# qasimyu/simuscop

Measured on AMD Instinct MI355X. Metric: simulated paired reads/sec (whole node) at 30x WGS PE150, higher is better.
Workload: dtype u32

## Files before the change

include/simuscop_amd.h:

```cpp
#ifndef SIMUSCOP_AMD_H
#define SIMUSCOP_AMD_H

#include <stdint.h>

#ifdef __cplusplus
extern "C" {
#endif

#define SG_OK 0
#define SG_ERR_INVALID 1
#define SG_ERR_HIP 2
#define SG_ERR_UNSUPPORTED 3
#define SG_ERR_OVERFLOW 4
#define SG_ERR_FORMAT 5

#define SG_MAX_EVENTS 32

typedef struct sg_ctx sg_ctx;

int sg_create(sg_ctx** ctx, int device, uint64_t seed);
void sg_destroy(sg_ctx* ctx);
void sg_release_cached_memory(void);
const char* sg_last_error(const sg_ctx* ctx);
int sg_set_stream(sg_ctx* ctx, void* hip_stream);
// ... 301 lines not shown
int sg_train_feed_bgzf(sg_ctx* ctx, const void* members, uint64_t bytes);
int sg_train_bam_info(sg_ctx* ctx, uint64_t* records, uint64_t* inflated_bytes, double* seconds);

int sg_emit_variant(sg_ctx* ctx);
#define SG_EMIT_STRAIGHT_LINE 1
#define SG_EMIT_GENERIC_K3_LDS 2
#define SG_EMIT_GENERIC_LDS 3
#define SG_EMIT_GENERIC_GLOBAL 4
typedef struct sg_emit_path_info {
  int32_t main_kernel;
  int32_t slow_rows_lds;
  uint32_t lds_bytes;
  uint32_t clean_cap;
} sg_emit_path_info;
int sg_emit_path(const sg_ctx* ctx, sg_emit_path_info* info);

uint64_t sg_cdf_count_le(double c);

int sg_sub_row_identity_first(const double cdf4[4], int cd, uint64_t cum[3], uint8_t order[4]);
uint32_t sg_row_symbols(const double* cdf, int n);
int sg_alias_row(const double* cdf, int n, uint32_t lgW, uint32_t* thr, uint8_t* lo, uint8_t* hi);

#define SG_VCF_SKIP 0
#define SG_VCF_SNV 1
#define SG_VCF_INS 2
#define SG_VCF_DEL 3
#define SG_VCF_MALFORMED 4
#define SG_VCF_UNDECIDED 5
#define SG_VCF_HOMO 1u
#define SG_VCF_KNOWN 2u
// ... 36 lines not shown
```

simuscop_amd/__init__.py:

```python
from __future__ import annotations

import ctypes as C
import os

PKG_DIR = os.path.dirname(os.path.abspath(__file__))
LIB_DIR = os.path.join(PKG_DIR, "lib")
ENGINE_SO = os.path.join(LIB_DIR, "libsimuscop_amd.so")
HOST_SO = os.path.join(LIB_DIR, "libsimuscop_host.so")
SIMUREADS = os.path.join(LIB_DIR, "simuReads")

SG_K_NAMES = ["plan", "namebase", "indel", "scan", "emit", "emit_slow"]

ENGINE_SYMBOLS = [
    "sg_create", "sg_destroy", "sg_last_error", "sg_set_stream", "sg_set_seed", "sg_set_strict_bases", "sg_load_profile",
    "sg_upload_haplotypes", "sg_reference_begin", "sg_reference_chunk", "sg_sync", "sg_reference_scan",
    "sg_reference_commit", "sg_build_haplotypes", "sg_haplotype_codes", "sg_compress", "sg_fetch_compressed", "sg_deflate_bgzf",
    "sg_bgzf_eof", "sg_deflate_plan", "sg_detach_outputs", "sg_outputs_sizes", "sg_outputs_fetch",
    "sg_outputs_last_error", "sg_release_outputs", "sg_plan", "sg_sample", "sg_result", "sg_fetch", "sg_device_output",
    "sg_gc_percent", "sg_set_profiling", "sg_kernel_times", "sg_emit_info", "sg_emit_variant", "sg_emit_path", "sg_cdf_count_le", "sg_fetch_range", "sg_host_alloc",
    "sg_sub_row_identity_first", "sg_row_symbols", "sg_alias_row", "sg_window_weights", "sg_windows_build", "sg_plan_windows", "sg_plan_range", "sg_windows_drop",
    "sg_host_free", "sg_profile_prepare", "sg_profile_tables_error", "sg_load_prepared_profile", "sg_profile_tables_free", "sg_train_count",
    "sg_train_begin", "sg_train_feed", "sg_train_capped", "sg_train_finish", "sg_train_end",
    "sg_bgzf_members", "sg_inflate_bgzf", "sg_train_bam_start", "sg_train_feed_bgzf", "sg_train_bam_info",
    "sg_release_cached_memory",
    "sg_truth_align", "sg_truth_map", "sg_truth_pieces", "sg_truth_reads", "sg_truth_bam", "sg_fetch_truth", "sg_truth_info",
    "sg_truth_bam_tags", "sg_truth_tag_info", "sg_truth_tags",
    "sg_bamsort_pass", "sg_bamsort_merge", "sg_bamsort_index", "sg_bamsort_fetch",
    "sg_bamindex_begin", "sg_bamindex_add", "sg_bamindex_chunks", "sg_bamindex_finish", "sg_bamindex_end",
    "sg_depth_begin", "sg_depth_add", "sg_depth_add_spans", "sg_depth_bins", "sg_depth_runs", "sg_depth_fetch", "sg_depth_reset",
    "sg_depth_info", "sg_depth_end",
    "sg_variants_begin", "sg_variants_add", "sg_variants_counts", "sg_variants_reset", "sg_variants_info", "sg_variants_end",
    "sg_variant_observe",
    "sg_errtab_begin", "sg_errtab_add", "sg_errtab_counts", "sg_errtab_reset", "sg_errtab_info", "sg_errtab_end", "sg_errtab_observe",
    "sg_vcf_begin", "sg_vcf_feed", "sg_vcf_feed_bgzf", "sg_vcf_undecided", "sg_vcf_finish", "sg_vcf_rows", "sg_vcf_end", "sg_vcf_row",
# ... 22 lines not shown

class SgProfileCdf(C.Structure):
    _fields_ = [("n_bases", C.c_int32), ("bases", C.c_char * 8), ("kmer", C.c_int32), ("bins", C.c_int32),
                ("read_length", C.c_int32), ("n_qual", C.c_int32), ("min_qual", C.c_int32),
                ("insert_rate", C.c_double), ("del_rate", C.c_double),
                ("ins_cdf", C.POINTER(C.c_double)), ("n_ins", C.c_int32),
                ("del_cdf", C.POINTER(C.c_double)), ("n_del", C.c_int32),
                ("subs_cdf1", C.POINTER(C.c_double)), ("subs_cdf2", C.POINTER(C.c_double)),
                ("qual_cdf", C.POINTER(C.c_double)), ("isize_cdf", C.POINTER(C.c_double)),
                ("n_isize", C.c_int32), ("isize_min", C.c_int32), ("insert_size", C.c_int32)]


class SgWindow(C.Structure):
    _fields_ = [("hap_base", C.c_uint64), ("chain", C.c_uint32), ("spos", C.c_uint32), ("len", C.c_uint32),
                ("n_reads", C.c_int32), ("seg", C.c_uint32), ("slot_base", C.c_uint32)]


class SgBatch(C.Structure):
    _fields_ = [("batch_id", C.c_uint32), ("paired", C.c_int32), ("name_prefix", C.c_char_p),
                ("windows", C.POINTER(SgWindow)), ("n_windows", C.c_uint64),
                ("seg_size", C.POINTER(C.c_uint32)), ("seg_first_window", C.POINTER(C.c_uint32)),
                ("n_segs", C.c_uint32), ("first_window", C.c_uint32), ("first_slot", C.c_uint32)]


class SgGcWindow(C.Structure):
    _fields_ = [("start", C.c_uint64), ("chain", C.c_uint32), ("len", C.c_uint32)]


class SgGcModel(C.Structure):
    _fields_ = [("means", C.POINTER(C.c_double)), ("std", C.c_double), ("quantiles", C.POINTER(C.c_double)), ("lg_cells", C.c_uint32),
# ... 175 lines not shown
    lib.sg_gc_percent.argtypes = [vp, C.POINTER(SgGcWindow), C.c_uint64, C.POINTER(C.c_int32)]
    lib.sg_window_weights.argtypes = [vp, C.POINTER(SgGcWindow), C.POINTER(C.c_uint32), C.POINTER(C.c_uint32), C.c_uint64, C.POINTER(SgGcModel),
                                      C.POINTER(C.c_double), C.POINTER(C.c_int32)]
    lib.sg_windows_build.argtypes = [vp, C.c_uint32, C.POINTER(SgWindowGen), C.c_uint64, C.c_uint32, C.POINTER(SgGcModel), C.POINTER(C.c_double),
                                     C.POINTER(C.c_uint64)]
    lib.sg_plan_windows.argtypes = [vp, C.c_uint32, C.POINTER(SgWindowGen), C.c_uint64, C.POINTER(SgActiveSeg), C.c_uint32, C.c_uint32, C.c_uint32,
                                    C.c_int32, C.c_char_p, C.POINTER(C.c_uint64), C.POINTER(C.c_uint64)]
    lib.sg_plan_range.argtypes = [vp, C.c_uint32, C.c_uint32]
    lib.sg_windows_drop.argtypes = [vp]
    lib.sg_windows_drop.restype = None
    lib.sg_set_profiling.argtypes = [vp, C.c_int]
    lib.sg_kernel_times.argtypes = [vp, C.POINTER(C.c_float)]
    lib.sg_emit_info.argtypes = [vp, C.POINTER(C.c_uint64), C.POINTER(C.c_int)]
    lib.sg_emit_variant.argtypes = [vp]
    lib.sg_emit_path.argtypes = [vp, C.POINTER(SgEmitPathInfo)]
    lib.sg_cdf_count_le.argtypes = [C.c_double]
    lib.sg_cdf_count_le.restype = C.c_uint64
    lib.sg_sub_row_identity_first.argtypes = [C.POINTER(C.c_double), C.c_int, C.POINTER(C.c_uint64), C.POINTER(C.c_uint8)]
    lib.sg_row_symbols.argtypes = [C.POINTER(C.c_double), C.c_int]
    lib.sg_row_symbols.restype = C.c_uint32
    lib.sg_alias_row.argtypes = [C.POINTER(C.c_double), C.c_int, C.c_uint32, C.POINTER(C.c_uint32), C.POINTER(C.c_uint8),
                                 C.POINTER(C.c_uint8)]
    lib.sg_truth_align.argtypes = [C.POINTER(SgTruthPiece), C.c_uint64, C.c_uint64, C.c_uint32, C.c_int, C.POINTER(C.c_uint32), C.c_uint32,
                                   C.POINTER(C.c_int32), C.POINTER(C.c_int64), C.POINTER(C.c_uint32), C.c_uint32, C.POINTER(C.c_uint32)]
    lib.sg_truth_map.argtypes = [vp, C.POINTER(SgHapPiece), C.c_char_p, C.c_uint64, C.POINTER(C.c_int32), C.c_uint32]
    lib.sg_truth_pieces.argtypes = [vp, C.c_uint32, C.POINTER(SgTruthPiece), C.c_uint64, C.POINTER(C.c_uint64)]
    lib.sg_truth_reads.argtypes = [vp, C.c_int, C.c_uint32, C.c_uint32, C.POINTER(SgTruthRead)]
    lib.sg_truth_bam.argtypes = [vp, C.POINTER(C.c_uint64), C.POINTER(C.c_uint64)]
    lib.sg_fetch_truth.argtypes = [vp, C.c_int, C.c_uint64, C.c_uint64, C.c_char_p]
    lib.sg_truth_info.argtypes = [vp, C.POINTER(C.c_uint64), C.POINTER(C.c_uint64)]
# ... 809 lines not shown
```

simuscop_amd/csrc/sg_api.cpp:

```cpp
#include <algorithm>
#include <cstdlib>
#include <cstring>

#include "sg_api.h"
#include "sg_profile_tables.h"

thread_local std::string g_create_error;

struct sg_outputs {
  int device = 0;
  hipStream_t stream = nullptr;
  OutputSet bufs;
  uint64_t text_bytes[2] = {0, 0}, gz_bytes[2] = {0, 0};
  std::string err;
  ~sg_outputs() {
    if (stream) { (void)hipStreamSynchronize(stream); (void)hipStreamDestroy(stream); }
  }
};

sg_ctx::~sg_ctx() {
  (void)hipSetDevice(device);
  if (stream) (void)hipStreamSynchronize(stream);
  for (sg_outputs* o : spare) delete o;
  if (evs_created)
    for (auto& ev : evs) (void)hipEventDestroy(ev);
  if (own_stream) { (void)hipStreamSynchronize(own_stream); (void)hipStreamDestroy(own_stream); }
  if (mail) (void)hipHostFree(mail);
}

int finish_plan(sg_ctx* ctx, uint64_t nw, uint32_t n_segs, uint32_t n_slots, uint32_t batch_id, uint32_t first_window,
                       uint32_t first_slot, int32_t paired, const char* name_prefix) {
  const size_t plen = name_prefix ? strlen(name_prefix) : 0;
  const uint32_t nm = paired ? 2 : 1;
  SG_ENSURE(ctx->prefix, plen + 16);
  SG_ENSURE(ctx->pairs, ((size_t)n_slots + 1) * sizeof(sg::PairRec));
  SG_ENSURE(ctx->win_actual, (nw + 1) * 4);
  SG_ENSURE(ctx->win_namebase, (nw + 1) * 4);
  SG_ENSURE(ctx->events, ((size_t)nm * n_slots + 1) * 4 * SG_MAX_EVENTS);
  SG_ENSURE(ctx->recoff, ((size_t)nm * n_slots + 1) * 4);
  SG_ENSURE(ctx->meta, ((size_t)nm * n_slots + 1) * 48);
  SG_ENSURE(ctx->totals, sg::kTotalsBytes);
  SG_ENSURE(ctx->bsum, ((size_t)nm * ((n_slots + 255) / 256) + 1) * 8);
  SG_HIP(hipMemcpyAsync(ctx->prefix.p, name_prefix, plen, hipMemcpyHostToDevice, ctx->stream));
  SG_HIP(hipStreamSynchronize(ctx->stream));

  sg::DevBatch& B = ctx->B;
  B.windows = ctx->windows.as<sg_window>();
  B.n_windows = nw;
  B.seg_size = ctx->segmeta.as<uint32_t>();
  B.seg_first_window = ctx->segmeta.as<uint32_t>() + n_segs;
  B.n_segs = n_segs;
  B.n_slots = n_slots;
  B.batch_id = batch_id;
  B.win_offset = first_window;
  B.slot_offset = first_slot;
  B.paired = paired ? 1 : 0;
  B.prefix = ctx->prefix.as<uint8_t>();
  B.prefix_len = (uint32_t)plen;
  for (int i = 0; i < 4; i++) B.prefix_w[i] = 0;
  for (size_t i = 0; i < plen && i < 16; i++) B.prefix_w[i / 4] |= (uint32_t)(uint8_t)name_prefix[i] << (8 * (i % 4));
  B.pairs = ctx->pairs.as<sg::PairRec>();
  B.win_actual = ctx->win_actual.as<uint32_t>();
  B.win_namebase = ctx->win_namebase.as<uint32_t>();
  B.events = ctx->events.as<uint32_t>();
  B.recloc = ctx->recoff.as<uint32_t>();
  B.blkbase = ctx->bsum.as<uint64_t>();
  B.seg_shift = sg::record_seg_shift((uint32_t)n_slots);
// ... 275 lines not shown
    uint64_t planned = x.n_reads <= 0 ? 0 : (b->paired ? ((uint64_t)x.n_reads + 1) / 2 : (uint64_t)x.n_reads);
    slots += planned;
    if (slots > 0xFFFFFFF0ull) return ctx->fail(SG_ERR_INVALID, "sg_plan: more than 2^32 fragments in one batch");
  }
  for (uint32_t s = 0; s < b->n_segs; s++)
    if (b->seg_first_window[s] > b->seg_first_window[s + 1] || b->seg_first_window[s + 1] > nw)
      return ctx->fail(SG_ERR_INVALID, "sg_plan: seg_first_window not monotone");
  if (b->n_segs && (b->seg_first_window[0] != 0 || b->seg_first_window[b->n_segs] != nw))
    return ctx->fail(SG_ERR_INVALID, "sg_plan: seg_first_window must cover all windows");
  const size_t plen = b->name_prefix ? strlen(b->name_prefix) : 0;
  if (plen == 0 || plen > 990) return ctx->fail(SG_ERR_INVALID, "sg_plan: bad name_prefix (1..990 bytes)");
  for (uint64_t w = 0; w < nw; w++) {
    const sg_window& x = b->windows[w];
    if (x.chain >= ctx->hap.len.size()) return ctx->fail(SG_ERR_INVALID, "sg_plan: window.chain out of range");
    if (x.hap_base + x.spos + x.len > ctx->hap.len[x.chain]) return ctx->fail(SG_ERR_INVALID, "sg_plan: window runs past its chain");
  }
  SG_ENSURE(ctx->windows, (nw + 1) * sizeof(sg_window));
  SG_ENSURE(ctx->segmeta, ((size_t)b->n_segs * 2 + 2) * 4);
  if (nw) SG_HIP(hipMemcpyAsync(ctx->windows.p, b->windows, nw * sizeof(sg_window), hipMemcpyHostToDevice, ctx->stream));
  if (b->n_segs) {
    SG_HIP(hipMemcpyAsync(ctx->segmeta.p, b->seg_size, (size_t)b->n_segs * 4, hipMemcpyHostToDevice, ctx->stream));
    SG_HIP(hipMemcpyAsync(ctx->segmeta.as<uint32_t>() + b->n_segs, b->seg_first_window, ((size_t)b->n_segs + 1) * 4,
                          hipMemcpyHostToDevice, ctx->stream));
  }
  return finish_plan(ctx, nw, b->n_segs, (uint32_t)slots, b->batch_id, b->first_window, b->first_slot, b->paired, b->name_prefix);
}

int sg_sample(sg_ctx* ctx) {
  if (int rc = sg_pass_need(ctx, "sg_sample", sg_ctx::Pass::Planned)) return rc;
  return run_pass(ctx);
}

int sg_emit_variant(sg_ctx* ctx) {
  if (!ctx || !ctx->have_profile) return -1;
  return sg::emit_variant(ctx->P);
}

int sg_emit_path(const sg_ctx* ctx, sg_emit_path_info* info) {
  if (!ctx || !info || ctx->pass.stage != sg_ctx::Pass::Settled) return SG_ERR_INVALID;
  const sg::EmitPath& path = ctx->pass.emit_path;
  *info = sg_emit_path_info{path.main_kernel, path.slow_rows_lds, path.lds_bytes, path.clean_cap};
  return SG_OK;
}

int sg_emit_info(sg_ctx* ctx, uint64_t* queued_items, int* requeued) {
  if (int rc = sg_pass_need(ctx, "sg_emit_info", sg_ctx::Pass::Settled)) return rc;
  if (queued_items) *queued_items = ctx->pass.slow_items;
  if (requeued) *requeued = ctx->pass.slow_overflow ? 1 : 0;
  return SG_OK;
}

int sg_result(sg_ctx* ctx, uint64_t* bytes_r1, uint64_t* bytes_r2, uint64_t* n_fragments) {
  if (int rc = sg_pass_need(ctx, "sg_result", sg_ctx::Pass::Settled, true)) return rc;
  const uint64_t* totals = ctx->pass.host_totals;
  if (bytes_r1) *bytes_r1 = totals[0];
  if (bytes_r2) *bytes_r2 = ctx->B.paired ? totals[1] : 0;
  if (n_fragments) *n_fragments = totals[2];
// ... 84 lines not shown
```

simuscop_amd/csrc/sg_api.h:

```cpp
#pragma once
#include <hip/hip_runtime.h>

#include <map>
#include <string>
#include <utility>
#include <vector>

#include "sg_device.h"
#include "sg_haplotypes.h"

struct DevBuf {
  void* p = nullptr;
  size_t cap = 0;
  int dev = 0;
  DevBuf() = default;
  DevBuf(DevBuf&& o) noexcept : p(std::exchange(o.p, nullptr)), cap(std::exchange(o.cap, 0)), dev(o.dev) {}
  DevBuf& operator=(DevBuf&& o) noexcept {
    if (this != &o) { release(); p = std::exchange(o.p, nullptr); cap = std::exchange(o.cap, 0); dev = o.dev; }
    return *this;
  }
  DevBuf(const DevBuf&) = delete;
  DevBuf& operator=(const DevBuf&) = delete;
  ~DevBuf() { release(); }
  int ensure(size_t bytes);
// ... 10 lines not shown

struct sg_outputs;
struct sg_train_session;

struct sg_ctx {
  int device = 0;
  hipStream_t own_stream = nullptr;
  hipStream_t stream = nullptr;
  uint64_t seed = 0;
  std::string err;

  bool have_profile = false, have_haps = false;
  sg::DevProfile P{};
  sg::DevBatch B{};
  OutputSet out;
  DevBuf tab, chains, chains2, chain_meta, windows, segmeta, prefix, pairs, win_actual, win_namebase, events, recoff, meta, totals, bsum,
      slowq, ref_raw, ref_codes, ref_meta, hap_work, gz_work,
      infl_src, infl_meta, infl_out, infl_crc,
      defl_src, defl_out;
  struct ChainLayout {
    std::vector<uint64_t> off, len;
    size_t total = 0;
  } hap;
  struct TruthInfo {
    uint64_t n_given = 0;
    bool from_build = false, mapped = false;
    std::vector<sg_truth_piece> sorted;
    std::vector<uint64_t> chain_first;
    uint32_t n_refs = 0;
  };
  struct Truth : TruthInfo {
// ... 55 lines not shown
    struct PlanInfo {
      bool valid = false;
      uint32_t n_active = 0, batch_id = 0;
      int32_t paired = 0;
      std::string prefix;
      std::vector<uint32_t> seg_first, seg_size;
      std::vector<uint64_t> slot_first;
    };
    std::map<uint32_t, Store> stores;
    DevBuf plan, work, gc, model;
    PlanInfo info;
  } win;
  uint64_t ref_raw_bytes = 0;
  sg_train_session* train = nullptr;
  std::vector<sg::DevContig> ref_contigs;
  uint64_t* mail = nullptr;
  struct Pass {
    enum Stage { None, Planned, Queued, Settled } stage;
    explicit Pass(Stage s = None) : stage(s) {}
    bool rows_current = true;
    bool speculative = false;
    uint64_t host_totals[4] = {0, 0, 0, 0};
    uint64_t host_flags[2] = {0, 0};
    uint64_t slow_items = 0;
    bool slow_overflow = false;
    sg::EmitPath emit_path = {0, -1, 0, 0};
    bool have_gz = false;
    uint64_t gz_bytes[2] = {0, 0};
    bool have_bam = false;
    bool bam_sorted = false;
// ... 17 lines not shown
#define SG_HIP(call)                                        \
  do {                                                      \
    hipError_t _e = (call);                                 \
    if (_e != hipSuccess) return ctx->hipfail(_e, #call);   \
  } while (0)
#define SG_ENSURE(buf, bytes)                                                                  \
  do {                                                                                         \
    int _e = (buf).ensure(bytes);                                                              \
    if (_e) return ctx->hipfail((hipError_t)_e, "hipMalloc(" #buf ")");                        \
  } while (0)

namespace sg { struct PieceMap; }
int sg_pass_prelude(sg_ctx* ctx, const char* who, sg::PieceMap* map, bool bam_names = false);
int sg_pass_need(sg_ctx* ctx, const char* who, sg_ctx::Pass::Stage at_least, bool settle_now = false);
int finish_plan(sg_ctx* ctx, uint64_t nw, uint32_t n_segs, uint32_t n_slots, uint32_t batch_id, uint32_t first_window,
                uint32_t first_slot, int32_t paired, const char* name_prefix);
void retire_plan(sg_ctx* ctx);
int deflate_text(sg_ctx* ctx, const uint8_t* text, uint64_t bytes, DevBuf& gz, uint64_t* gz_total, const char* who);
int sg_pass_records(sg_ctx* ctx, const char* who, uint32_t tags, bool sorted, uint64_t* record_bytes, uint64_t* bgzf_bytes);
namespace sg { struct TruthJob; }
int bamsort_pass_keys(sg_ctx* ctx, const sg::TruthJob& J, bool paired);
int bamsort_pass_order(sg_ctx* ctx, const sg::TruthJob& J, uint64_t* rec_off, uint64_t* total);
struct SgSortBufs {
  DevBuf* keys;
  DevBuf* vals;
  int* cur;
  uint32_t* hist;
  uint64_t* hist_off;
  uint64_t* bsum;
  uint64_t* total;
};
// ... 46 lines not shown
```

simuscop_amd/csrc/sg_api_windows.cpp:

```cpp
#include <cstring>

#include "sg_api.h"
#include "sg_scan.h"
#include "sg_windows.h"

namespace {

int bad(sg_ctx* ctx, const char* who, const std::string& what) { return ctx->fail(SG_ERR_INVALID, std::string(who) + ": " + what); }

int check_model(sg_ctx* ctx, const sg_gc_model* m, const char* who) { return m->lg_cells < 1 || m->lg_cells > 20 || !m->frag_size ? bad(ctx, who, "bad model") : SG_OK; }
int upload_model(sg_ctx* ctx, const sg_gc_model* m, sg_gc_model* dev) {
  const size_t cells = (size_t)1 << m->lg_cells;
  SG_ENSURE(ctx->win.model, (101 + cells + 1) * 8);
  double* d = ctx->win.model.as<double>();
  SG_HIP(hipMemcpyAsync(d, m->means, 101 * 8, hipMemcpyHostToDevice, ctx->stream));
  SG_HIP(hipMemcpyAsync(d + 101, m->quantiles, (cells + 1) * 8, hipMemcpyHostToDevice, ctx->stream));
  *dev = {d, m->std, d + 101, m->lg_cells, m->frag_size, m->full_tile_form, m->ctx24};
  return SG_OK;
}
int check_windows(sg_ctx* ctx, const sg_gc_window* windows, uint64_t n, const char* who) {
  for (uint64_t w = 0; w < n; w++) {
    if (windows[w].chain >= ctx->hap.len.size()) return bad(ctx, who, "chain out of range");
    if (windows[w].start + windows[w].len > ctx->hap.len[windows[w].chain]) return bad(ctx, who, "window runs past its chain");
  }
// ... 164 lines not shown
int sg_plan_range(sg_ctx* ctx, uint32_t a0, uint32_t a1) {
  if (!ctx) return SG_ERR_INVALID;
  const sg_ctx::Windows::PlanInfo& pi = ctx->win.info;
  if (!pi.valid) return ctx->fail(SG_ERR_INVALID, "sg_plan_range: call sg_plan_windows first");
  if (a0 >= a1 || a1 > pi.n_active) return ctx->fail(SG_ERR_INVALID, "sg_plan_range: empty or out-of-range run of segments");
  SG_HIP(hipSetDevice(ctx->device));
  const uint32_t w_lo = pi.seg_first[a0], w_hi = pi.seg_first[a1], n_segs = a1 - a0;
  const uint64_t nw = (uint64_t)w_hi - w_lo;
  const uint64_t slot_lo = pi.slot_first[a0], slots = pi.slot_first[a1] - slot_lo;
  SG_ENSURE(ctx->windows, (nw + 1) * sizeof(sg_window));
  SG_ENSURE(ctx->segmeta, ((size_t)n_segs * 2 + 2) * 4);
  std::vector<uint32_t> segmeta;
  for (uint32_t a = a0; a < a1; a++) segmeta.push_back(pi.seg_size[a]);
  for (uint32_t a = a0; a <= a1; a++) segmeta.push_back(pi.seg_first[a] - w_lo);
  SG_HIP(hipMemcpyAsync(ctx->segmeta.p, segmeta.data(), segmeta.size() * 4, hipMemcpyHostToDevice, ctx->stream));
  sg::launch_slice(ctx->win.plan.as<sg_window>(), w_lo, nw, a0, (uint32_t)slot_lo, ctx->windows.as<sg_window>(), ctx->stream);
  SG_HIP(hipGetLastError());
  return finish_plan(ctx, nw, n_segs, (uint32_t)slots, pi.batch_id, w_lo, (uint32_t)slot_lo, pi.paired, pi.prefix.c_str());
}

}
```

simuscop_amd/csrc/sg_device.h:

```cpp
#pragma once
#include <hip/hip_runtime.h>
#include <stdint.h>

#include "../../include/simuscop_amd.h"

namespace sg {

constexpr size_t kTotalsSegBase = 128 + 2 * 2 * 8 * 128;
constexpr size_t kTotalsBytes = kTotalsSegBase + 2 * 16 * 8 + 64;

constexpr int kBaseRounds = 7;

enum : uint32_t { KIND_HAP = 1, KIND_GC = 2, KIND_PLAN = 3, KIND_INDEL = 4, KIND_AUX = 5, KIND_BASE = 6 };

struct PairRec {
  uint32_t win;
  uint32_t namepos;
  uint32_t fl;
  uint32_t k;
  uint64_t foff;
  uint64_t pad;
};

__host__ __device__ inline uint32_t ev_pack(uint32_t j, uint32_t len, uint32_t del) { return j | (len << 16) | (del << 31); }

struct DevProfile {
  const uint4* sub;
  uint32_t sub_mate_rows;
  const uint2* alias;
  uint32_t lgW;
  const uint32_t* fast_lds;
  uint32_t fast_mate_words;
  uint32_t fast_stride;
  const uint4* fast_sub;
  const uint2* fast_alias;
  const uint32_t* ins_row; uint32_t ins_lg;
  const uint32_t* del_row; uint32_t del_lg;
// ... 11 lines not shown

struct DevBatch {
  const uint8_t* chains;
  const uint64_t* chain_off;
  const uint64_t* chain_len;
  const uint8_t* chains2_fwd;
  const uint8_t* chains2_rc;
  const uint16_t* chains_bad;
  uint64_t chains_total;
  const sg_window* windows;
  uint64_t n_windows;
  const uint32_t* seg_size;
  const uint32_t* seg_first_window;
  uint32_t n_segs;
  uint32_t n_slots;
  uint32_t batch_id;
  uint32_t win_offset, slot_offset;
  int32_t paired;
  const uint8_t* prefix;
  uint32_t prefix_len;
  uint32_t prefix_w[4];
  uint32_t k0, k1;
  uint32_t diag;
  uint32_t strict_bases;
  PairRec* pairs;
  uint32_t* win_actual;
  uint32_t* win_namebase;
  uint32_t* events;
  uint32_t* recloc;
  uint64_t* blkbase;
// ... 27 lines not shown
```

simuscop_amd/csrc/sg_kernels.hip:

```cpp
#include <algorithm>
#include <cstdlib>
#include <type_traits>

#include "sg_emit.h"

namespace sg {

__device__ __forceinline__ uint32_t row_search(const uint32_t* __restrict__ row, uint32_t lg, uint32_t x) {
  const uint32_t* T = row + 1;
  uint32_t pos = 0;
  for (uint32_t step = lg ? (1u << (lg - 1)) : 0; step; step >>= 1)
    if (x > T[pos + step - 1]) pos += step;
  return row[0] + pos;
}

#define PLAN_S 16

__device__ __forceinline__ bool plan_attempt(const DevProfile& P, const DevBatch& B, const sg_window& win, uint64_t w,
                                             uint32_t attempt, uint64_t clen, uint32_t c3, PairRec& r, const uint32_t* isz_row,
                                             uint32_t seg_size, uint64_t chain_off) {
  uint32_t x[4];
  philox4x32_10((uint32_t)w + B.win_offset, attempt, 0, c3, B.k0, B.k1, x);
  const double frac = __dmul_rn((double)x[0], 1.0 / 4294967296.0);
  const double v = __dadd_rn((double)win.spos, __dmul_rn((double)win.len, frac));
  const uint32_t pos = (uint32_t)(long long)v;
  uint32_t isz;
  if (B.paired) isz = isz_row ? (uint32_t)P.isz_min + row_search(isz_row, P.isz_lg, x[1]) : (uint32_t)P.fixed_isz;
  else isz = win.len;
  const uint64_t avail = clen - (win.hap_base + pos);
  const uint32_t flen = avail < (uint64_t)isz ? (uint32_t)avail : isz;
  const uint32_t strand = B.paired ? 0u : (x[2] >> 31);
  r.win = (uint32_t)w; r.fl = flen | (strand << 31);
  r.namepos = pos % seg_size;
  r.foff = chain_off + win.hap_base + pos;
  r.pad = 0;
  return flen >= (uint32_t)P.L;
}

__global__ __launch_bounds__(256) void plan_kernel(DevProfile P, DevBatch B) {
  __shared__ uint32_t isz_lds[1025];
  const uint32_t* isz_row = P.isz_row;
  if (P.isz_row && P.isz_lg <= 10u) {
    for (uint32_t i = threadIdx.x; i < (1u << P.isz_lg) + 1u; i += blockDim.x) isz_lds[i] = P.isz_row[i];
    isz_row = isz_lds;
  }
  __syncthreads();
  if (blockIdx.x == 0)
    for (uint32_t i = threadIdx.x; i < kTotalsBytes / 4u; i += blockDim.x) ((uint32_t*)B.totals)[i] = 0u;
  const uint64_t gid = (uint64_t)blockIdx.x * blockDim.x + threadIdx.x;
  const uint64_t w = gid / PLAN_S;
  const uint32_t j = (uint32_t)(gid % PLAN_S);
  if (w >= B.n_windows) return;
  const sg_window win = B.windows[w];
  const int n = win.n_reads;
  const uint32_t planned = n <= 0 ? 0u : (B.paired ? ((uint32_t)n + 1u) / 2u : (uint32_t)n);
  const uint64_t clen = B.chain_len[win.chain];
  const uint32_t seg_size = B.seg_size[win.seg];
  const uint64_t chain_off = B.chain_off[win.chain];
  const uint32_t c3 = dev_ctx(KIND_PLAN, 0, B.batch_id);
  const uint64_t last_start = win.hap_base + win.spos + win.len - 1u;
  const uint64_t need = B.paired ? (uint64_t)P.isz_hi : (uint64_t)win.len;
  const uint32_t shortest = B.paired ? (uint32_t)P.isz_lo : win.len;
  const bool safe = last_start + need <= clen && shortest >= (uint32_t)P.L;
  if (safe) {
    for (uint32_t k = j; k < planned; k += PLAN_S) {
      PairRec r;
      plan_attempt(P, B, win, w, k, clen, c3, r, isz_row, seg_size, chain_off);
      r.k = k;
      B.pairs[win.slot_base + k] = r;
    }
    if (j == 0) B.win_actual[w] = planned;
    return;
  }
  if (j != 0) return;
  uint32_t done = 0, fail = 0, attempt = 0;
  while (done < planned) {
    PairRec r;
    if (!plan_attempt(P, B, win, w, attempt++, clen, c3, r, isz_row, seg_size, chain_off)) {
      if (++fail > 1000) break;
      continue;
    }
    r.k = done;
    B.pairs[win.slot_base + done] = r;
    done++;
  }
  for (uint32_t k = done; k < planned; k++) {
    PairRec r;
    r.win = (uint32_t)w; r.namepos = 0; r.fl = 0; r.k = k; r.foff = 0; r.pad = 0;
    B.pairs[win.slot_base + k] = r;
  }
  B.win_actual[w] = done;
}

__global__ __launch_bounds__(64) void namebase_kernel(DevBatch B) {
  const uint32_t s = blockIdx.x;
  const uint32_t lane = threadIdx.x;
  const uint32_t w0 = B.seg_first_window[s], w1 = B.seg_first_window[s + 1];
  uint32_t carry = 0;
  for (uint32_t base = w0; base < w1; base += 64) {
    uint32_t w = base + lane;
    uint32_t v = w < w1 ? B.win_actual[w] : 0u;
    uint32_t incl = v;
#pragma unroll
    for (int d = 1; d < 64; d <<= 1) {
      uint32_t t = __shfl_up(incl, d);
      if ((int)lane >= d) incl += t;
    }
    if (w < w1) B.win_namebase[w] = carry + incl - v;
    carry += __shfl(incl, 63);
  }
  if (lane == 0) atomicAdd((unsigned long long*)&B.totals[2], (unsigned long long)carry);
}

__global__ __launch_bounds__(256) void indel_kernel(DevProfile P, DevBatch B) {
  __shared__ uint4 row_lds[256 * 3];
  __shared__ uint16_t cand[512];
  __shared__ uint32_t cand_n;
  __shared__ uint2 found[2][256];
  __shared__ uint32_t found_first[2][256];
  __shared__ uint32_t wave_len[2][4];
  const uint32_t tid = threadIdx.x, lane = tid & 63u, wv = tid >> 6;
  const uint32_t t = blockIdx.x * blockDim.x + tid;
  const uint32_t nm = B.paired ? 2u : 1u;
  uint4* const wave_rows = row_lds + (tid & ~63u) * 3u;
  uint4* const my_row = wave_rows + lane * 3u;
  const uint32_t t_wave = t - lane;
// ... 2 lines not shown
  if ((uint32_t)P.L + 1u <= 256u) {
    for (uint32_t i = tid; i <= (uint32_t)P.L; i += blockDim.x) gap_lds[i] = P.gap_row[i];
    gap = gap_lds;
  }
  if (tid == 0u) cand_n = 0u;
  const bool in_batch = t < B.n_slots;
  PairRec rec = {};
  if (in_batch) rec = B.pairs[t];
  const uint32_t flen = rec.fl & 0x7FFFFFFFu;
  const bool live = flen != 0u;
  const uint32_t L = (uint32_t)P.L;
  uint32_t fragcount = 0, touches_bad[2] = {0, 0};
  const uint64_t foff = rec.foff;
  const uint32_t rev1 = rec.fl >> 31;
  if (live) {
    fragcount = B.win_namebase[rec.win] + rec.k + 1u;
    for (uint32_t m = 0; m < nm; m++) {
      const bool rev = B.paired ? (m == 1u) : (rev1 != 0u);
      const uint64_t t0 = (rev ? foff + flen - L : foff) - 8u, t1 = t0 + L + 24u;
      uint32_t bad = 0;
      for (uint64_t b = t0 >> 6; b <= (t1 >> 6); b++) bad |= (B.chains_bad[b >> 4] >> (b & 15u)) & 1u;
      touches_bad[m] = bad;
    }
  }
  __syncthreads();
  for (uint32_t m = 0; m < nm; m++) {
    found[m][tid] = make_uint2(0u, 0u);
    found_first[m][tid] = 0u;
    bool has = false;
    if (live) {
      uint32_t x4[4];
// ... 101 lines not shown
      const uint32_t rev = B.paired ? m : rev1;
      mid = ReadRow::make_m1(flen, touches_bad[m], rev, np, nev, hdr, nev == 1u ? found_first[m][tid] : 0u);
    }
    my_row[1] = mid;
    if (t_wave < B.n_slots) {
      wave_lds_sync();
      uint4* dst = B.meta + ((size_t)m * B.n_slots + t_wave) * 3;
      const uint32_t n_pieces = min(B.n_slots - t_wave, 64u) * 3u;
#pragma unroll
      for (uint32_t i = 0; i < 3u; i++) {
        const uint32_t q = i * 64u + lane;
        if (q < n_pieces) dst[q] = wave_rows[q];
      }
    }
  }
  uint32_t incl[2];
  for (uint32_t m = 0; m < nm; m++) {
    uint32_t v = rl[m];
#pragma unroll
    for (int d = 1; d < 64; d <<= 1) {
      const uint32_t up = __shfl_up(v, d, 64);
      if ((int)lane >= d) v += up;
    }
    incl[m] = v;
    if (lane == 63u) wave_len[m][wv] = v;
  }
  __syncthreads();
  for (uint32_t m = 0; m < nm; m++) {
    uint32_t base = 0, all = 0;
#pragma unroll
// ... 51 lines not shown
  if (threadIdx.x == 0) {
    __hip_atomic_store(&segbase[j], buf[1023], __ATOMIC_RELAXED, __HIP_MEMORY_SCOPE_AGENT);
    __threadfence();
    ticket = atomicAdd(arrived, 1u);
  }
  __syncthreads();
  if (ticket + 1u == gridDim.x && threadIdx.x == 0) {
    __threadfence();
    uint64_t acc = 0;
    for (uint32_t i = 0; i < gridDim.x; i++) {
      const uint64_t v = __hip_atomic_load(&segbase[i], __ATOMIC_RELAXED, __HIP_MEMORY_SCOPE_AGENT);
      __hip_atomic_store(&segbase[i], acc, __ATOMIC_RELAXED, __HIP_MEMORY_SCOPE_AGENT);
      acc += v;
    }
    B.totals[m] = acc;
  }
}


__device__ __forceinline__ uint32_t template_code(uint32_t raw, bool rev, bool x_known) {
  return raw < 4u ? (rev ? raw ^ 2u : raw) : ((raw == 6u && !rev && x_known) ? 6u : 4u);
}

__device__ __noinline__ uint64_t slow_codes(const uint8_t* frag, uint32_t flen, uint32_t rev, const uint32_t* ev,
                                            uint32_t nev, uint32_t np, uint32_t i0, uint32_t K, uint32_t slot,
                                            uint32_t ctx_aux, uint32_t k0, uint32_t k1, bool x_known) {
  uint64_t out = 0;
  uint32_t e = 0;
  int shift = 0;
  uint32_t nextw = nev ? ev[0] : 0xFFFFFFFFu;
// ... 294 lines not shown
  }
}

__global__ void mail_kernel(const uint64_t* __restrict__ totals, uint64_t* __restrict__ mail) {
  if (threadIdx.x < 5u) mail[threadIdx.x] = totals[threadIdx.x];
}
void launch_mail(const uint64_t* totals, uint64_t* mail, hipStream_t s) {
  hipLaunchKernelGGL(mail_kernel, dim3(1), dim3(64), 0, s, totals, mail);
}
void launch_plan(const DevProfile& P, const DevBatch& B, hipStream_t s) {
  if (!B.n_windows) return;
  uint32_t grid = (uint32_t)((B.n_windows * PLAN_S + 255) / 256);
  hipLaunchKernelGGL(plan_kernel, dim3(grid), dim3(256), 0, s, P, B);
}
void launch_namebase(const DevBatch& B, hipStream_t s) {
  if (!B.n_segs) return;
  hipLaunchKernelGGL(namebase_kernel, dim3(B.n_segs), dim3(64), 0, s, B);
}
void launch_indel(const DevProfile& P, const DevBatch& B, hipStream_t s) {
  if (!B.n_slots) return;
  hipLaunchKernelGGL(indel_kernel, dim3((B.n_slots + 255) / 256), dim3(256), 0, s, P, B);
}
void launch_header(const DevProfile& P, const DevBatch& B, hipStream_t s) {
  if (!B.n_slots) return;
  const bool fast = emit_uses_fast_kernel(P, B);
  if (fast && B.prefix_len <= 16u) return;
  dim3 grid((B.n_slots + 255) / 256, B.paired ? 2 : 1);
  hipLaunchKernelGGL(header_kernel, grid, dim3(256), 0, s, B);
}
uint32_t record_seg_shift(uint32_t n_slots) {
  const uint32_t nblk = (n_slots + 255u) >> 8;
// ... 103 lines not shown
```

simuscop_amd/csrc/sg_windows.h:

```cpp
#pragma once
#include <hip/hip_runtime.h>
#include <stdint.h>

#include "../../include/simuscop_amd.h"

namespace sg {

struct WindowList { sg_gc_window* win; uint32_t* seg_ord; uint32_t* win_ord; int32_t* gc; };
struct GenList { sg_window_gen* gens; uint64_t* prefix; uint32_t n_gens; };
struct BuildWork { GenList g; uint64_t* seg_first; WindowList w; double* seg_sum; };
struct PlanWork {
  GenList g;
  sg_active_seg* act;
  uint32_t *seg_first, *planned;
  unsigned long long* seg_sum;
  uint64_t *off, *bsum, *total, *seg_slots;
};

void launch_gc(const uint8_t* chains, const uint64_t* chain_off, const sg_gc_window* wins, uint64_t n, int32_t* out, hipStream_t s);
void launch_weights(const uint8_t* chains, const uint64_t* chain_off, const WindowList& w, uint64_t n, const sg_gc_model& m, uint64_t seed,
                    double* out, hipStream_t s);
void launch_tile(const BuildWork& b, uint64_t n, uint32_t frag, hipStream_t s);
void launch_seg_sum(const double* wt, const uint64_t* seg_first, uint32_t n_segs, double* out, hipStream_t s);
void launch_plan_rows(const PlanWork& p, uint64_t n, uint32_t frag, const double* wt, uint32_t n_act, sg_window* rows, int32_t paired,
                      hipStream_t s);
void launch_slice(const sg_window* all, uint64_t w_lo, uint64_t n, uint32_t a0, uint32_t slot_lo, sg_window* out, hipStream_t s);

}
```

simuscop_amd/csrc/sg_windows.hip:

```cpp
#include "sg_philox.h"
#include "sg_scan.h"
#include "sg_windows.h"

namespace sg {

__device__ __forceinline__ uint32_t count_eq_bytes(uint32_t w, uint32_t c) {
  uint32_t x = w ^ (c * 0x01010101u);
  uint32_t t = (x & 0x7F7F7F7Fu) + 0x7F7F7F7Fu;
  t = ~(t | x | 0x7F7F7F7Fu);
  return __popc(t);
}

__global__ __launch_bounds__(256) void gc_kernel(const uint8_t* __restrict__ chains, const uint64_t* __restrict__ chain_off,
                                                 const sg_gc_window* __restrict__ wins, uint64_t n, int32_t* __restrict__ out) {
  const uint64_t w = (uint64_t)blockIdx.x * (blockDim.x / 64) + (threadIdx.x >> 6);
  const uint32_t lane = threadIdx.x & 63;
  if (w >= n) return;
  const sg_gc_window win = wins[w];
  const uint8_t* p = chains + chain_off[win.chain] + win.start;
  uint32_t gc = 0, nn = 0;
  for (uint32_t b = lane * 16; b < win.len; b += 64 * 16) {
    uint32_t v[4];
    __builtin_memcpy(v, p + b, 16);
    const uint32_t rem = win.len - b;
// ... 135 lines not shown
  if (w >= n) return;
  const int32_t r = rows[w].n_reads;
  planned[w] = r <= 0 ? 0u : (paired ? ((uint32_t)r + 1u) / 2u : (uint32_t)r);
}
__global__ __launch_bounds__(256) void slot_base_kernel(sg_window* __restrict__ rows, uint64_t n, const uint64_t* __restrict__ off) {
  const uint64_t w = (uint64_t)blockIdx.x * blockDim.x + threadIdx.x;
  if (w < n) rows[w].slot_base = (uint32_t)off[w];
}
__global__ __launch_bounds__(64) void seg_slots_kernel(const uint64_t* __restrict__ off, const uint32_t* __restrict__ seg_first, uint32_t n_act,
                                                       const uint64_t* __restrict__ total, uint64_t* __restrict__ out) {
  const uint32_t a = blockIdx.x * blockDim.x + threadIdx.x;
  if (a < n_act) out[a] = off[seg_first[a]];
  if (a == n_act) out[a] = *total;
}
__global__ __launch_bounds__(256) void slice_kernel(const sg_window* __restrict__ all, uint64_t w_lo, uint64_t n, uint32_t a0, uint32_t slot_lo,
                                                    sg_window* __restrict__ out) {
  const uint64_t w = (uint64_t)blockIdx.x * blockDim.x + threadIdx.x;
  if (w >= n) return;
  sg_window o = all[w_lo + w];
  o.seg -= a0;
  o.slot_base -= slot_lo;
  out[w] = o;
}
static inline uint32_t blocks256(uint64_t n) { return (uint32_t)((n + 255) / 256); }
void launch_gc(const uint8_t* chains, const uint64_t* chain_off, const sg_gc_window* wins, uint64_t n, int32_t* out, hipStream_t s) {
  if (n) hipLaunchKernelGGL(gc_kernel, dim3((uint32_t)((n + 3) / 4)), dim3(256), 0, s, chains, chain_off, wins, n, out);
}
void launch_weights(const uint8_t* chains, const uint64_t* chain_off, const WindowList& w, uint64_t n, const sg_gc_model& m, uint64_t seed,
                    double* out, hipStream_t s) {
  if (!n) return;
  launch_gc(chains, chain_off, w.win, n, w.gc, s);
  hipLaunchKernelGGL(gc_weight_kernel, dim3(blocks256(n)), dim3(256), 0, s, w.gc, w.win, w.seg_ord, w.win_ord, n, m.means, m.std, m.quantiles,
                     m.lg_cells, m.frag_size, m.full_tile_form, KIND_GC | (m.ctx24 << 8), (uint32_t)seed, (uint32_t)(seed >> 32), out);
}
void launch_tile(const BuildWork& b, uint64_t n, uint32_t frag, hipStream_t s) {
  if (n) hipLaunchKernelGGL(tile_kernel, dim3(blocks256(n)), dim3(256), 0, s, b.g.gens, b.g.prefix, b.g.n_gens, n, frag, b.seg_first, b.w.win,
                            b.w.seg_ord, b.w.win_ord);
}
void launch_seg_sum(const double* wt, const uint64_t* seg_first, uint32_t n_segs, double* out, hipStream_t s) {
  if (n_segs) hipLaunchKernelGGL(seg_sum_kernel, dim3(n_segs), dim3(256), 0, s, wt, seg_first, n_segs, out);
}
void launch_plan_rows(const PlanWork& p, uint64_t n, uint32_t frag, const double* wt, uint32_t n_act, sg_window* rows, int32_t paired,
                      hipStream_t s) {
  if (!n) return;
  hipLaunchKernelGGL(window_reads_kernel, dim3(blocks256(n)), dim3(256), 0, s, p.g.gens, p.g.prefix, p.g.n_gens, n, frag, wt, p.act, rows, p.seg_sum);
  hipLaunchKernelGGL(seg_remainder_kernel, dim3((n_act + 63) / 64), dim3(64), 0, s, p.act, p.seg_first, n_act, p.seg_sum, rows);
  hipLaunchKernelGGL(planned_kernel, dim3(blocks256(n)), dim3(256), 0, s, rows, n, paired, p.planned);
  launch_scan_u32(p.planned, (uint32_t)n, p.bsum, p.off, p.total, s);
  hipLaunchKernelGGL(slot_base_kernel, dim3(blocks256(n)), dim3(256), 0, s, rows, n, p.off);
  hipLaunchKernelGGL(seg_slots_kernel, dim3((n_act + 64) / 64), dim3(64), 0, s, p.off, p.seg_first, n_act, p.total, p.seg_slots);
}
void launch_slice(const sg_window* all, uint64_t w_lo, uint64_t n, uint32_t a0, uint32_t slot_lo, sg_window* out, hipStream_t s) {
  if (n) hipLaunchKernelGGL(slice_kernel, dim3(blocks256(n)), dim3(256), 0, s, all, w_lo, n, a0, slot_lo, out);
}

}
```

Baseline: 2.145 billion.

## Replace namebase prefix-scan kernel with short-window correction list

```diff
diff --git a/include/simuscop_amd.h b/include/simuscop_amd.h
--- a/include/simuscop_amd.h
+++ b/include/simuscop_amd.h
@@ -339,6 +339,12 @@
   uint32_t clean_cap;
 } sg_emit_path_info;
 int sg_emit_path(const sg_ctx* ctx, sg_emit_path_info* info);
+#define SG_SHORT_LIST_CAP 32
+int sg_fragment_numbering(const sg_ctx* ctx, uint32_t* n_short);
+typedef struct sg_short_window { uint32_t win, seg_end, planned; } sg_short_window;
+uint64_t sg_short_windows(const sg_window* windows, uint64_t n_windows, const uint32_t* seg_first_window, uint32_t n_segs,
+                          const uint64_t* chain_len, int32_t paired, uint32_t isz_lo, uint32_t read_length, sg_short_window* out,
+                          uint64_t cap);
 
 uint64_t sg_cdf_count_le(double c);
 
diff --git a/simuscop_amd/__init__.py b/simuscop_amd/__init__.py
--- a/simuscop_amd/__init__.py
+++ b/simuscop_amd/__init__.py
@@ -17,7 +17,7 @@
     "sg_reference_commit", "sg_build_haplotypes", "sg_haplotype_codes", "sg_compress", "sg_fetch_compressed", "sg_deflate_bgzf",
     "sg_bgzf_eof", "sg_deflate_plan", "sg_detach_outputs", "sg_outputs_sizes", "sg_outputs_fetch",
     "sg_outputs_last_error", "sg_release_outputs", "sg_plan", "sg_sample", "sg_result", "sg_fetch", "sg_device_output",
-    "sg_gc_percent", "sg_set_profiling", "sg_kernel_times", "sg_emit_info", "sg_emit_variant", "sg_emit_path", "sg_cdf_count_le", "sg_fetch_range", "sg_host_alloc",
+    "sg_gc_percent", "sg_set_profiling", "sg_kernel_times", "sg_emit_info", "sg_emit_variant", "sg_emit_path", "sg_fragment_numbering", "sg_short_windows", "sg_cdf_count_le", "sg_fetch_range", "sg_host_alloc",
     "sg_sub_row_identity_first", "sg_row_symbols", "sg_alias_row", "sg_window_weights", "sg_windows_build", "sg_plan_windows", "sg_plan_range", "sg_windows_drop",
     "sg_host_free", "sg_profile_prepare", "sg_profile_tables_error", "sg_load_prepared_profile", "sg_profile_tables_free", "sg_train_count",
     "sg_train_begin", "sg_train_feed", "sg_train_capped", "sg_train_finish", "sg_train_end",
@@ -70,6 +70,10 @@
 class SgWindow(C.Structure):
     _fields_ = [("hap_base", C.c_uint64), ("chain", C.c_uint32), ("spos", C.c_uint32), ("len", C.c_uint32),
                 ("n_reads", C.c_int32), ("seg", C.c_uint32), ("slot_base", C.c_uint32)]
+
+
+class SgShortWindow(C.Structure):
+    _fields_ = [("win", C.c_uint32), ("seg_end", C.c_uint32), ("planned", C.c_uint32)]
 
 
 class SgBatch(C.Structure):
@@ -275,6 +279,10 @@
     lib.sg_emit_info.argtypes = [vp, C.POINTER(C.c_uint64), C.POINTER(C.c_int)]
     lib.sg_emit_variant.argtypes = [vp]
     lib.sg_emit_path.argtypes = [vp, C.POINTER(SgEmitPathInfo)]
+    lib.sg_fragment_numbering.argtypes = [vp, C.POINTER(C.c_uint32)]
+    lib.sg_short_windows.argtypes = [C.POINTER(SgWindow), C.c_uint64, C.POINTER(C.c_uint32), C.c_uint32, C.POINTER(C.c_uint64), C.c_int32,
+                                     C.c_uint32, C.c_uint32, C.POINTER(SgShortWindow), C.c_uint64]
+    lib.sg_short_windows.restype = C.c_uint64
     lib.sg_cdf_count_le.argtypes = [C.c_double]
     lib.sg_cdf_count_le.restype = C.c_uint64
     lib.sg_sub_row_identity_first.argtypes = [C.POINTER(C.c_double), C.c_int, C.POINTER(C.c_uint64), C.POINTER(C.c_uint8)]
diff --git a/simuscop_amd/csrc/sg_api.cpp b/simuscop_amd/csrc/sg_api.cpp
--- a/simuscop_amd/csrc/sg_api.cpp
+++ b/simuscop_amd/csrc/sg_api.cpp
@@ -29,7 +29,7 @@
 }
 
 int finish_plan(sg_ctx* ctx, uint64_t nw, uint32_t n_segs, uint32_t n_slots, uint32_t batch_id, uint32_t first_window,
-                       uint32_t first_slot, int32_t paired, const char* name_prefix) {
+                       uint32_t first_slot, int32_t paired, const char* name_prefix, uint64_t n_short) {
   const size_t plen = name_prefix ? strlen(name_prefix) : 0;
   const uint32_t nm = paired ? 2 : 1;
   SG_ENSURE(ctx->prefix, plen + 16);
@@ -51,6 +51,12 @@
   B.seg_first_window = ctx->segmeta.as<uint32_t>() + n_segs;
   B.n_segs = n_segs;
   B.n_slots = n_slots;
+  uint64_t short_cap = sg::kShortListCap;
+  if (const char* e = getenv("SG_SHORT_LIST_CAP")) short_cap = std::min<uint64_t>(short_cap, strtoull(e, nullptr, 10));
+  B.short_list = ctx->short_list.as<sg::ShortWindow>();
+  B.use_namebase = n_short > short_cap ? 1u : 0u;
+  B.n_short = B.use_namebase ? 0u : (uint32_t)n_short;
+  ctx->n_short = n_short;
   B.batch_id = batch_id;
   B.win_offset = first_window;
   B.slot_offset = first_slot;
@@ -356,6 +362,8 @@
     const sg_window& x = b->windows[w];
     if (x.chain >= ctx->hap.len.size()) return ctx->fail(SG_ERR_INVALID, "sg_plan: window.chain out of range");
     if (x.hap_base + x.spos + x.len > ctx->hap.len[x.chain]) return ctx->fail(SG_ERR_INVALID, "sg_plan: window runs past its chain");
+    if (w < b->seg_first_window[x.seg] || w >= b->seg_first_window[x.seg + 1])
+      return ctx->fail(SG_ERR_INVALID, "sg_plan: window.seg is not the segment seg_first_window puts the window in");
   }
   SG_ENSURE(ctx->windows, (nw + 1) * sizeof(sg_window));
   SG_ENSURE(ctx->segmeta, ((size_t)b->n_segs * 2 + 2) * 4);
@@ -365,7 +373,12 @@
     SG_HIP(hipMemcpyAsync(ctx->segmeta.as<uint32_t>() + b->n_segs, b->seg_first_window, ((size_t)b->n_segs + 1) * 4,
                           hipMemcpyHostToDevice, ctx->stream));
   }
-  return finish_plan(ctx, nw, b->n_segs, (uint32_t)slots, b->batch_id, b->first_window, b->first_slot, b->paired, b->name_prefix);
+  sg_short_window list[sg::kShortListCap];
+  const uint64_t n_short = sg_short_windows(b->windows, nw, b->seg_first_window, b->n_segs, ctx->hap.len.data(), b->paired, (uint32_t)ctx->P.isz_lo,
+                                            (uint32_t)ctx->P.L, list, sg::kShortListCap);
+  SG_ENSURE(ctx->short_list, sizeof(list) + 64);
+  if (n_short) SG_HIP(hipMemcpyAsync(ctx->short_list.p, list, sizeof(list), hipMemcpyHostToDevice, ctx->stream));
+  return finish_plan(ctx, nw, b->n_segs, (uint32_t)slots, b->batch_id, b->first_window, b->first_slot, b->paired, b->name_prefix, n_short);
 }
 
 int sg_sample(sg_ctx* ctx) {
@@ -383,6 +396,28 @@
   const sg::EmitPath& path = ctx->pass.emit_path;
   *info = sg_emit_path_info{path.main_kernel, path.slow_rows_lds, path.lds_bytes, path.clean_cap};
   return SG_OK;
+}
+
+int sg_fragment_numbering(const sg_ctx* ctx, uint32_t* n_short) {
+  if (!ctx || ctx->pass.stage < sg_ctx::Pass::Planned || !ctx->pass.rows_current) return -1;
+  if (n_short) *n_short = (uint32_t)std::min<uint64_t>(ctx->n_short, 0xFFFFFFFFu);
+  return (int)ctx->B.use_namebase;
+}
+
+uint64_t sg_short_windows(const sg_window* windows, uint64_t n_windows, const uint32_t* seg_first_window, uint32_t n_segs,
+                          const uint64_t* chain_len, int32_t paired, uint32_t isz_lo, uint32_t read_length, sg_short_window* out,
+                          uint64_t cap) {
+  uint64_t n = 0;
+  if (!n_windows || !windows || !seg_first_window || !chain_len) return 0;
+  for (uint32_t s = 0; s < n_segs; s++)
+    for (uint64_t w = seg_first_window[s]; w + 1 < seg_first_window[s + 1]; w++) {
+      const sg_window& x = windows[w];
+      if (!sg::window_can_fall_short(x, chain_len[x.chain], paired != 0, isz_lo, read_length)) continue;
+      const uint32_t planned = x.n_reads <= 0 ? 0u : (paired ? ((uint32_t)x.n_reads + 1u) / 2u : (uint32_t)x.n_reads);
+      if (out && n < cap) out[n] = sg_short_window{(uint32_t)w, seg_first_window[s + 1], planned};
+      n++;
+    }
+  return n;
 }
 
 int sg_emit_info(sg_ctx* ctx, uint64_t* queued_items, int* requeued) {
diff --git a/simuscop_amd/csrc/sg_api.h b/simuscop_amd/csrc/sg_api.h
--- a/simuscop_amd/csrc/sg_api.h
+++ b/simuscop_amd/csrc/sg_api.h
@@ -48,7 +48,7 @@
   sg::DevProfile P{};
   sg::DevBatch B{};
   OutputSet out;
-  DevBuf tab, chains, chains2, chain_meta, windows, segmeta, prefix, pairs, win_actual, win_namebase, events, recoff, meta, totals, bsum,
+  DevBuf tab, chains, chains2, chain_meta, windows, segmeta, prefix, pairs, win_actual, win_namebase, short_list, events, recoff, meta, totals, bsum,
       slowq, ref_raw, ref_codes, ref_meta, hap_work, gz_work,
       infl_src, infl_meta, infl_out, infl_crc,
       defl_src, defl_out;
@@ -134,6 +134,7 @@
   uint64_t ref_raw_bytes = 0;
   sg_train_session* train = nullptr;
   std::vector<sg::DevContig> ref_contigs;
+  uint64_t n_short = 0;
   uint64_t* mail = nullptr;
   struct Pass {
     enum Stage { None, Planned, Queued, Settled } stage;
@@ -181,7 +182,7 @@
 int sg_pass_prelude(sg_ctx* ctx, const char* who, sg::PieceMap* map, bool bam_names = false);
 int sg_pass_need(sg_ctx* ctx, const char* who, sg_ctx::Pass::Stage at_least, bool settle_now = false);
 int finish_plan(sg_ctx* ctx, uint64_t nw, uint32_t n_segs, uint32_t n_slots, uint32_t batch_id, uint32_t first_window,
-                uint32_t first_slot, int32_t paired, const char* name_prefix);
+                uint32_t first_slot, int32_t paired, const char* name_prefix, uint64_t n_short);
 void retire_plan(sg_ctx* ctx);
 int deflate_text(sg_ctx* ctx, const uint8_t* text, uint64_t bytes, DevBuf& gz, uint64_t* gz_total, const char* who);
 int sg_pass_records(sg_ctx* ctx, const char* who, uint32_t tags, bool sorted, uint64_t* record_bytes, uint64_t* bgzf_bytes);
diff --git a/simuscop_amd/csrc/sg_api_windows.cpp b/simuscop_amd/csrc/sg_api_windows.cpp
--- a/simuscop_amd/csrc/sg_api_windows.cpp
+++ b/simuscop_amd/csrc/sg_api_windows.cpp
@@ -202,9 +202,16 @@
   for (uint32_t a = a0; a < a1; a++) segmeta.push_back(pi.seg_size[a]);
   for (uint32_t a = a0; a <= a1; a++) segmeta.push_back(pi.seg_first[a] - w_lo);
   SG_HIP(hipMemcpyAsync(ctx->segmeta.p, segmeta.data(), segmeta.size() * 4, hipMemcpyHostToDevice, ctx->stream));
-  sg::launch_slice(ctx->win.plan.as<sg_window>(), w_lo, nw, a0, (uint32_t)slot_lo, ctx->windows.as<sg_window>(), ctx->stream);
-  SG_HIP(hipGetLastError());
-  return finish_plan(ctx, nw, n_segs, (uint32_t)slots, pi.batch_id, w_lo, (uint32_t)slot_lo, pi.paired, pi.prefix.c_str());
-}
-
-}
+  SG_ENSURE(ctx->short_list, sizeof(sg::ShortWindow) * sg::kShortListCap + 64);
+  sg::ShortWindow* const short_list = ctx->short_list.as<sg::ShortWindow>();
+  uint32_t* const counted = (uint32_t*)(short_list + sg::kShortListCap);
+  uint32_t n_short = 0;
+  SG_HIP(hipMemsetAsync(counted, 0, 4, ctx->stream));
+  const sg::ShortRule rule{pi.paired, (uint32_t)ctx->P.isz_lo, (uint32_t)ctx->P.L};
+  sg::launch_slice(ctx->win.plan.as<sg_window>(), w_lo, nw, a0, (uint32_t)slot_lo, ctx->windows.as<sg_window>(),
+                   ctx->segmeta.as<uint32_t>() + n_segs, ctx->B.chain_len, rule, short_list, counted, ctx->stream);
+  if (int rc = sg_read_back(ctx, &n_short, counted, 4)) return rc;
+  return finish_plan(ctx, nw, n_segs, (uint32_t)slots, pi.batch_id, w_lo, (uint32_t)slot_lo, pi.paired, pi.prefix.c_str(), n_short);
+}
+
+}
diff --git a/simuscop_amd/csrc/sg_device.h b/simuscop_amd/csrc/sg_device.h
--- a/simuscop_amd/csrc/sg_device.h
+++ b/simuscop_amd/csrc/sg_device.h
@@ -7,6 +7,7 @@
 namespace sg {
 
 constexpr size_t kTotalsSegBase = 128 + 2 * 2 * 8 * 128;
+constexpr size_t kTotalsDeadSlots = kTotalsSegBase + 2 * 16 * 8 + 8;
 constexpr size_t kTotalsBytes = kTotalsSegBase + 2 * 16 * 8 + 64;
 
 constexpr int kBaseRounds = 7;
@@ -19,8 +20,18 @@
   uint32_t fl;
   uint32_t k;
   uint64_t foff;
-  uint64_t pad;
+  uint32_t seg_k;
+  uint32_t unused;
 };
+
+using ShortWindow = ::sg_short_window;
+constexpr uint32_t kShortListCap = SG_SHORT_LIST_CAP;
+
+__host__ __device__ inline bool window_can_fall_short(const sg_window& win, uint64_t clen, bool paired, uint32_t isz_lo, uint32_t L) {
+  const uint64_t last_start = win.hap_base + win.spos + win.len - 1u;
+  const uint32_t shortest = paired ? isz_lo : win.len;
+  return !(last_start + L <= clen && shortest >= L);
+}
 
 __host__ __device__ inline uint32_t ev_pack(uint32_t j, uint32_t len, uint32_t del) { return j | (len << 16) | (del << 31); }
 
@@ -62,6 +73,9 @@
   const uint32_t* seg_first_window;
   uint32_t n_segs;
   uint32_t n_slots;
+  const ShortWindow* short_list;
+  uint32_t n_short;
+  uint32_t use_namebase;
   uint32_t batch_id;
   uint32_t win_offset, slot_offset;
   int32_t paired;
diff --git a/simuscop_amd/csrc/sg_kernels.hip b/simuscop_amd/csrc/sg_kernels.hip
--- a/simuscop_amd/csrc/sg_kernels.hip
+++ b/simuscop_amd/csrc/sg_kernels.hip
@@ -33,7 +33,7 @@
   r.win = (uint32_t)w; r.fl = flen | (strand << 31);
   r.namepos = pos % seg_size;
   r.foff = chain_off + win.hap_base + pos;
-  r.pad = 0;
+  r.unused = 0;
   return flen >= (uint32_t)P.L;
 }
 
@@ -58,15 +58,14 @@
   const uint32_t seg_size = B.seg_size[win.seg];
   const uint64_t chain_off = B.chain_off[win.chain];
   const uint32_t c3 = dev_ctx(KIND_PLAN, 0, B.batch_id);
-  const uint64_t last_start = win.hap_base + win.spos + win.len - 1u;
-  const uint64_t need = B.paired ? (uint64_t)P.isz_hi : (uint64_t)win.len;
-  const uint32_t shortest = B.paired ? (uint32_t)P.isz_lo : win.len;
-  const bool safe = last_start + need <= clen && shortest >= (uint32_t)P.L;
+  const uint32_t seg_slot = win.slot_base - B.windows[B.seg_first_window[win.seg]].slot_base;
+  const bool safe = !window_can_fall_short(win, clen, B.paired != 0, (uint32_t)P.isz_lo, (uint32_t)P.L);
   if (safe) {
     for (uint32_t k = j; k < planned; k += PLAN_S) {
       PairRec r;
       plan_attempt(P, B, win, w, k, clen, c3, r, isz_row, seg_size, chain_off);
       r.k = k;
+      r.seg_k = seg_slot + k;
       B.pairs[win.slot_base + k] = r;
     }
     if (j == 0) B.win_actual[w] = planned;
@@ -81,12 +80,13 @@
       continue;
     }
     r.k = done;
+    r.seg_k = seg_slot + done;
     B.pairs[win.slot_base + done] = r;
     done++;
   }
   for (uint32_t k = done; k < planned; k++) {
     PairRec r;
-    r.win = (uint32_t)w; r.namepos = 0; r.fl = 0; r.k = k; r.foff = 0; r.pad = 0;
+    r.win = (uint32_t)w; r.namepos = 0; r.fl = 0; r.k = k; r.foff = 0; r.seg_k = 0; r.unused = 0;
     B.pairs[win.slot_base + k] = r;
   }
   B.win_actual[w] = done;
@@ -109,7 +109,6 @@
     if (w < w1) B.win_namebase[w] = carry + incl - v;
     carry += __shfl(incl, 63);
   }
-  if (lane == 0) atomicAdd((unsigned long long*)&B.totals[2], (unsigned long long)carry);
 }
 
 __global__ __launch_bounds__(256) void indel_kernel(DevProfile P, DevBatch B) {
@@ -142,7 +141,15 @@
   const uint64_t foff = rec.foff;
   const uint32_t rev1 = rec.fl >> 31;
   if (live) {
-    fragcount = B.win_namebase[rec.win] + rec.k + 1u;
+    if (B.use_namebase) {
+      fragcount = B.win_namebase[rec.win] + rec.k + 1u;
+    } else {
+      fragcount = rec.seg_k + 1u;
+      for (uint32_t i = 0; i < B.n_short; i++) {
+        const ShortWindow sw = B.short_list[i];
+        if (rec.win > sw.win && rec.win < sw.seg_end) fragcount -= sw.planned - B.win_actual[sw.win];
+      }
+    }
     for (uint32_t m = 0; m < nm; m++) {
       const bool rev = B.paired ? (m == 1u) : (rev1 != 0u);
       const uint64_t t0 = (rev ? foff + flen - L : foff) - 8u, t1 = t0 + L + 24u;
@@ -274,6 +281,10 @@
       }
     }
   }
+  {
+    const unsigned long long dead = __ballot(in_batch && !live);
+    if (dead && lane == 0u) atomicAdd((uint32_t*)((uint8_t*)B.totals + kTotalsDeadSlots), (uint32_t)__popcll(dead));
+  }
   uint32_t incl[2];
   for (uint32_t m = 0; m < nm; m++) {
     uint32_t v = rl[m];
@@ -355,6 +366,7 @@
       acc += v;
     }
     B.totals[m] = acc;
+    if (m == 0u) B.totals[2] = B.n_slots - *(const uint32_t*)((const uint8_t*)B.totals + kTotalsDeadSlots);
   }
 }
 
@@ -679,7 +691,7 @@
   hipLaunchKernelGGL(plan_kernel, dim3(grid), dim3(256), 0, s, P, B);
 }
 void launch_namebase(const DevBatch& B, hipStream_t s) {
-  if (!B.n_segs) return;
+  if (!B.n_segs || !B.use_namebase) return;
   hipLaunchKernelGGL(namebase_kernel, dim3(B.n_segs), dim3(64), 0, s, B);
 }
 void launch_indel(const DevProfile& P, const DevBatch& B, hipStream_t s) {
diff --git a/simuscop_amd/csrc/sg_windows.h b/simuscop_amd/csrc/sg_windows.h
--- a/simuscop_amd/csrc/sg_windows.h
+++ b/simuscop_amd/csrc/sg_windows.h
@@ -3,6 +3,7 @@
 #include <stdint.h>
 
 #include "../../include/simuscop_amd.h"
+#include "sg_device.h"
 
 namespace sg {
 
@@ -24,6 +25,8 @@
 void launch_seg_sum(const double* wt, const uint64_t* seg_first, uint32_t n_segs, double* out, hipStream_t s);
 void launch_plan_rows(const PlanWork& p, uint64_t n, uint32_t frag, const double* wt, uint32_t n_act, sg_window* rows, int32_t paired,
                       hipStream_t s);
-void launch_slice(const sg_window* all, uint64_t w_lo, uint64_t n, uint32_t a0, uint32_t slot_lo, sg_window* out, hipStream_t s);
+struct ShortRule { int32_t paired; uint32_t isz_lo, L; };
+void launch_slice(const sg_window* all, uint64_t w_lo, uint64_t n, uint32_t a0, uint32_t slot_lo, sg_window* out, const uint32_t* seg_first,
+                  const uint64_t* chain_len, const ShortRule& rule, ShortWindow* short_list, uint32_t* n_short, hipStream_t s);
 
 }
diff --git a/simuscop_amd/csrc/sg_windows.hip b/simuscop_amd/csrc/sg_windows.hip
--- a/simuscop_amd/csrc/sg_windows.hip
+++ b/simuscop_amd/csrc/sg_windows.hip
@@ -173,13 +173,21 @@
   if (a == n_act) out[a] = *total;
 }
 __global__ __launch_bounds__(256) void slice_kernel(const sg_window* __restrict__ all, uint64_t w_lo, uint64_t n, uint32_t a0, uint32_t slot_lo,
-                                                    sg_window* __restrict__ out) {
+                                                    sg_window* __restrict__ out, const uint32_t* __restrict__ seg_first,
+                                                    const uint64_t* __restrict__ chain_len, ShortRule rule, ShortWindow* __restrict__ short_list,
+                                                    uint32_t* n_short) {
   const uint64_t w = (uint64_t)blockIdx.x * blockDim.x + threadIdx.x;
   if (w >= n) return;
   sg_window o = all[w_lo + w];
   o.seg -= a0;
   o.slot_base -= slot_lo;
   out[w] = o;
+  const uint32_t seg_end = seg_first[o.seg + 1u];
+  if (w + 1u < seg_end && window_can_fall_short(o, chain_len[o.chain], rule.paired != 0, rule.isz_lo, rule.L)) {
+    const uint32_t i = atomicAdd(n_short, 1u);
+    const uint32_t planned = o.n_reads <= 0 ? 0u : (rule.paired ? ((uint32_t)o.n_reads + 1u) / 2u : (uint32_t)o.n_reads);
+    if (i < kShortListCap) short_list[i] = ShortWindow{(uint32_t)w, seg_end, planned};
+  }
 }
 static inline uint32_t blocks256(uint64_t n) { return (uint32_t)((n + 255) / 256); }
 void launch_gc(const uint8_t* chains, const uint64_t* chain_off, const sg_gc_window* wins, uint64_t n, int32_t* out, hipStream_t s) {
@@ -209,8 +217,9 @@
   hipLaunchKernelGGL(slot_base_kernel, dim3(blocks256(n)), dim3(256), 0, s, rows, n, p.off);
   hipLaunchKernelGGL(seg_slots_kernel, dim3((n_act + 64) / 64), dim3(64), 0, s, p.off, p.seg_first, n_act, p.total, p.seg_slots);
 }
-void launch_slice(const sg_window* all, uint64_t w_lo, uint64_t n, uint32_t a0, uint32_t slot_lo, sg_window* out, hipStream_t s) {
-  if (n) hipLaunchKernelGGL(slice_kernel, dim3(blocks256(n)), dim3(256), 0, s, all, w_lo, n, a0, slot_lo, out);
-}
-
-}
+void launch_slice(const sg_window* all, uint64_t w_lo, uint64_t n, uint32_t a0, uint32_t slot_lo, sg_window* out, const uint32_t* seg_first,
+                  const uint64_t* chain_len, const ShortRule& rule, ShortWindow* short_list, uint32_t* n_short, hipStream_t s) {
+  if (n) hipLaunchKernelGGL(slice_kernel, dim3(blocks256(n)), dim3(256), 0, s, all, w_lo, n, a0, slot_lo, out, seg_first, chain_len, rule, short_list, n_short);
+}
+
+}
```

Result: no change. 2.166 billion (median of 6 runs) (+1.0%).
